# yigolden/JpegLibrary

Hardware: AMD Instinct MI355X
Metric: Mpixels/s decoded, 4K 4:2:0 baseline Q75 RST=4, 1 & 8 GPU vs CPU ref (higher is better)
Workload: dtype f32; 1 GPU; 1024 x 3840x2160 420 baseline Q75 DRI=4 per GPU, output interleaved_u8 resident in HBM; images_per_gpu=1024

## Files before the change

jpeglibrary_amd/csrc/common.h:

```cpp
#pragma once
#include <stdint.h>

namespace jpgpu {

constexpr int kMaxScanComponents = 4;
constexpr int kMaxBlocksPerMcu = 16;
constexpr int kHuffLutBits = 9;
constexpr int kHuffLutSize = 1 << kHuffLutBits;
constexpr int kMaxHuffSlots = 8;

struct alignas(16) DevHuffTable {
    uint16_t lut[kHuffLutSize];
    uint16_t maxcode[18];
    uint8_t valoffset[20];
    uint8_t values[256];
    uint8_t pad[8];
};
static_assert(sizeof(DevHuffTable) % 16 == 0, "DevHuffTable must be a multiple of 16 bytes");

struct alignas(16) DevQuantTable {
    uint16_t q[64];
};

struct DevScanComponent {
    uint8_t component_index;
    uint8_t h, v;
    uint8_t hs, vs;
    uint8_t quant_slot;
    uint8_t dc_slot, ac_slot;
};

enum OutputFormat : int32_t { kFmtInterleavedU8 = 0, kFmtPlanarU8 = 1, kFmtPlanarI16 = 2, kFmtRgbU8 = 3, kFmtRgbaU8 = 4, kFmtExtendedU16 = 5, kFmtInterleavedU8Scaled = 6, kFmtRgbPlanarU8 = 7, kFmtRgbPlanarF16 = 8, kFmtRgbPlanarF32 = 9 };
constexpr int kNumOutputFormats = 10;
constexpr bool fmt_is_sample_bytes(int f) { return f == kFmtInterleavedU8 || f == kFmtInterleavedU8Scaled; }
constexpr bool fmt_is_rgb_planes(int f) { return f == kFmtRgbPlanarU8 || f == kFmtRgbPlanarF16 || f == kFmtRgbPlanarF32; }
constexpr bool fmt_is_rgb(int f) { return f == kFmtRgbU8 || f == kFmtRgbaU8 || fmt_is_rgb_planes(f); }
constexpr int fmt_rgb_plane_sample_bytes(int f) { return f == kFmtRgbPlanarF16 ? 2 : (f == kFmtRgbPlanarF32 ? 4 : 1); }
constexpr bool fmt_is_interleaved(int f) { return fmt_is_sample_bytes(f) || fmt_is_rgb(f); }
constexpr int fmt_bytes_per_pixel_rgb(int f) { return f == kFmtRgbaU8 ? 4 : 3; }

struct YccRgbFactors {
    int32_t cr_r, cr_g, cb_b, cb_g;
};
struct OutputAffine {
    float scale[3], bias[3];
};
constexpr OutputAffine kOutputAffineIdentity = {{1.0f, 1.0f, 1.0f}, {0.0f, 0.0f, 0.0f}};
enum ColorKind : int32_t { kColorGray = 0, kColorYcbcr = 1, kColorRgb = 2, kColorCmyk = 3, kColorYcck = 4 };
constexpr bool color_kind_by_file(int k) { return k == kColorRgb || k == kColorCmyk || k == kColorYcck; }
constexpr int color_kind_sample_bytes(int k) { return k == kColorGray ? 1 : (k == kColorCmyk || k == kColorYcck ? 4 : 3); }

struct alignas(16) DevScan {
    uint64_t data_off;
    uint64_t coef_off;
    uint64_t out_off;
    uint64_t plane_off[kMaxScanComponents];
    uint32_t plane_pitch[kMaxScanComponents];
    uint32_t data_len;
    uint32_t dri;
    uint32_t total_mcus, mcus_per_line, mcus_per_column;
    uint32_t n_intervals;
    uint32_t ends_off;
    uint32_t image_index;
    uint32_t level_shift;
    uint16_t width, height;
    uint8_t precision, frame_components, scan_components, max_h, max_v, blocks_per_mcu;
    uint8_t restart_check_at_end;
    uint8_t shadow_mask;
    DevScanComponent comp[kMaxScanComponents];
    uint8_t blk_comp[kMaxBlocksPerMcu];
    uint8_t blk_x[kMaxBlocksPerMcu];
    uint8_t blk_y[kMaxBlocksPerMcu];
    uint16_t huff_pool[kMaxHuffSlots];
    uint16_t quant_pool[kMaxScanComponents];
    uint64_t reserved0;
// ... 132 lines not shown
```

jpeglibrary_amd/csrc/device_batch_layout.cpp:

```cpp
#include "device_batch.h"

#include <hip/hip_runtime.h>
#include <stdio.h>
#include <stdlib.h>
#include <string.h>

#include <algorithm>
#include <vector>

#include "kernels.h"

namespace jpgpu {

static inline uint64_t align_up(uint64_t v, uint64_t a) { return (v + a - 1) / a * a; }

namespace {
template <typename T>
void xcd_interleave(std::vector<T> &w, int xcds) {
    if (xcds <= 1 || w.size() < (size_t)xcds * 8) return;
    const size_t n = w.size(), per = (n + xcds - 1) / xcds;
    std::vector<T> m;
    m.reserve(n);
    for (size_t i = 0; m.size() < n; i++) {
        const size_t src = (i % xcds) * per + i / xcds;
        if (src < n) m.push_back(w[src]);
    }
    w.swap(m);
}

struct LayoutSwitches {
    int dbg_delay_scan = -1, dbg_delay_ms = 0;
    bool dbg_status = false, prog_no_pipeline = false, no_subseq = false;
    uint32_t subseq_shift = 0;
    uint32_t stream_max_intervals = 16;
    uint32_t prog_spin_budget = 1u << 17;
    bool subseq_host_check = false;
    bool handoff_set = false, handoff_dense = false;
    bool tile_align = true;
    bool overlap = false;
    int xcds = 8;
    bool prog_by_scan = false, no_wave_chains = false, k1_three_pass = false;
};

LayoutSwitches read_layout_switches() {
    auto set = [](const char *name) { return getenv(name) != nullptr; };
    static const bool by_scan = set("JPGPU_PROG_BY_SCAN"), no_wave_chains = set("JPGPU_PROG_NO_WAVE_CHAINS"), three_pass = set("JPGPU_K1_THREE_PASS");
    LayoutSwitches sw;
    const char *dd = getenv("JPGPU_DEBUG_DELAY_SCAN");
    if (dd && sscanf(dd, "%d:%d", &sw.dbg_delay_scan, &sw.dbg_delay_ms) != 2) sw.dbg_delay_scan = -1;
    sw.dbg_status = set("JPGPU_DEBUG_STATUS");
    if (const char *ev = getenv("JPGPU_SUBSEQ_SHIFT")) sw.subseq_shift = (uint32_t)std::min(14, std::max(8, atoi(ev)));
    if (const char *ev = getenv("JPGPU_PROG_STREAM_MAX_INTERVALS")) sw.stream_max_intervals = (uint32_t)atoi(ev);
    sw.prog_no_pipeline = set("JPGPU_PROG_NO_PIPELINE");
    if (const char *ev = getenv("JPGPU_PROG_SPIN_BUDGET")) sw.prog_spin_budget = (uint32_t)strtoul(ev, nullptr, 10);
    sw.subseq_host_check = set("JPGPU_SUBSEQ_HOST_CHECK");
    if (const char *ev = getenv("JPGPU_DENSE_HANDOFF")) sw.handoff_set = true, sw.handoff_dense = atoi(ev) != 0;
    if (const char *ev = getenv("JPGPU_TILE_ALIGN")) sw.tile_align = atoi(ev) != 0;
    sw.no_subseq = set("JPGPU_NO_SUBSEQ");
    if (const char *ev = getenv("JPGPU_OVERLAP")) sw.overlap = atoi(ev) != 0;
    if (const char *ev = getenv("JPGPU_XCD_MAP")) sw.xcds = atoi(ev);
    sw.prog_by_scan = by_scan, sw.no_wave_chains = no_wave_chains, sw.k1_three_pass = three_pass;
    return sw;
// ... 99 lines not shown
    sub_same_valid_ = k2s_unchecked_ = k2s_idct_behind_ = false;
    k2s_host_checked_ = p.sw.subseq_host_check || keep_canvas_;
    dispose_jobs_.clear();
    split_scans_.clear();
    dispose_max_blocks_ = split_max_blocks_ = 0;
    dense_valid_ = dense_override_ = false;
    compressed_bytes_ = total_pixels_ = 0;
    for (uint32_t &b : k2_ticket_base_) b = 0;
    decodes_since_query_ = 0;
}

void DeviceBatch::choose_batch_shapes(UploadPlan &p) {
    uint64_t dri0_bits = 0;
    for (size_t j = 0; j < jobs_.size(); j++)
        if (jobs_[j].kind == kScanSequential && jobs_[j].geo.restart_interval == 0) dri0_bits += (uint64_t)jobs_[j].entropy_len * 8;
    while (p.subseq_shift < 12 && (dri0_bits >> p.subseq_shift) >= 500000u) p.subseq_shift++;
    while (p.subseq_shift > 9 && (dri0_bits >> p.subseq_shift) < 4096u) p.subseq_shift--;
    if (p.sw.subseq_shift) p.subseq_shift = p.sw.subseq_shift;
    uint64_t blocks = 0;
    for (const ScanJob &job : jobs_)
        if (job.kind != kScanProgressive) blocks += (uint64_t)job.geo.mcus_per_line * job.geo.mcus_per_column * (uint64_t)std::max(1, job.blocks_per_mcu);
    const uint64_t tiles = blocks / (uint64_t)kIdctBlocksPerWg + 1, want_wgs = 3ull * (uint64_t)(ctx_->num_cus > 0 ? ctx_->num_cus : 256);
    while (p.idct_tiles_per_wg > 1 && tiles / p.idct_tiles_per_wg < want_wgs) p.idct_tiles_per_wg /= 2;
    n_huff_slots_ = 1;
    for (const ScanJob &job : jobs_) n_huff_slots_ = std::max(n_huff_slots_, job.n_huff);
    k2_tab_bytes_ = kK2AcTabBytes + kK2DcTabBytes;
    for (const ScanJob &job : jobs_) {
        if (job.kind != kScanSequential) continue;
        uint32_t bytes = 0;
        for (int k = 0; k < job.n_huff; k++) {
            bool is_dc = false;
            for (int c = 0; c < job.scan_components; c++) is_dc |= job.dc_slot[c] == k;
            bytes += is_dc ? kK2DcTabBytes : kK2AcTabBytes;
        }
        k2_tab_bytes_ = std::max(k2_tab_bytes_, bytes);
    }
    p.huff_intervals_per_wg = 64u * (uint32_t)huffman_waves(k2_tab_bytes_);
}

uint16_t DeviceBatch::huff_index(UploadPlan &p, const HuffTable &t) {
    for (size_t i = 0; i < p.huff_keys.size(); i++)
        if (p.huff_keys[i]->num_values == t.num_values && memcmp(p.huff_keys[i]->bits, t.bits, 16) == 0 &&
            memcmp(p.huff_keys[i]->values, t.values, t.num_values) == 0)
            return (uint16_t)i;
    DevHuffTable d;
    t.to_device(&d);
    p.huff_keys.push_back(&t);
    huff_pool_.push_back(d);
    return (uint16_t)(huff_pool_.size() - 1);
}
uint16_t DeviceBatch::quant_index(const QuantTable &t) {
    DevQuantTable d;
    memcpy(d.q, t.elements, sizeof d.q);
    for (size_t i = 0; i < quant_pool_.size(); i++)
        if (memcmp(&quant_pool_[i], &d, sizeof d) == 0) return (uint16_t)i;
    quant_pool_.push_back(d);
    return (uint16_t)(quant_pool_.size() - 1);
}

void DeviceBatch::plan_image(UploadPlan &p, size_t ii, const std::vector<size_t> &file_len) {
    ImagePlan &img = images_[ii];
    img.out_offset = p.out_off;
    img.planes_offset = p.planes_off;
    img.coef_offset = p.coef_off;
    img.total_blocks = 0;
    if (img.status != JPGPU_OK) return;
    p.out_off = align_up(p.out_off + slot_bytes(img), 256);
    p.planes_off = align_up(p.planes_off + img.planes_bytes, 256);
    if (!img.jobs.empty()) total_pixels_ += (uint64_t)img.width * img.height;
    bool overlapping_scans = false;
    uint32_t seen = 0;
    for (int j : img.jobs) {
        const ScanJob &job = jobs_[j];
        if (job.kind != kScanSequential || job.disabled) continue;
        overlapping_scans |= (component_mask(job) & seen) != 0;
        seen |= component_mask(job);
    }
    for (int j : img.jobs) {
        const ScanJob &job = jobs_[j];
        fill_scan(p, ii, j, file_len[ii]);
        if (job.kind == kScanFrameOnly && job.dispose_generic) plan_dispose_job(j, !img.replay_skip);
        if (job.kind == kScanProgressive) {
            if (!job.disabled && !img.replay_skip) plan_progressive_scan(p, img, j);
            continue;
        }
        plan_entropy_work(p, ii, j);
        if (img.replay_skip) continue;
        if (h_scans_[j].blocks_per_mcu == 0) continue;
        plan_idct_work(p, ii, j, overlapping_scans);
    }
}

void DeviceBatch::fill_scan(UploadPlan &p, size_t ii, int j, size_t file_len) {
    const ImagePlan &img = images_[ii];
    const ScanJob &job = jobs_[j];
    DevScan &s = h_scans_[j];
    memset(&s, 0, sizeof s);
    const BaselineGeometry &g = job.geo;
    s.kind = (uint8_t)job.kind;
    s.last_interval = job.last_interval;
    s.data_off = img.file_offset + job_entropy_off_[j];
    s.data_len = (uint32_t)(file_len - job_entropy_off_[j]);
    if (job.kind == kScanFrameOnly) s.data_len = 0;
    if (job.kind == kScanProgressive) {
        const size_t end = find_scan_end(job.entropy, job.entropy_len);
        s.data_len = (uint32_t)std::min<size_t>(end + 2, job.entropy_len);
// ... 594 lines not shown
```

jpeglibrary_amd/csrc/k3_idct.hip:

```cpp
#include <hip/hip_runtime.h>
#include <stdint.h>

#include <algorithm>
#include <atomic>
#include <cstdio>
#include <cstdlib>

#include "common.h"
#include "kernels.h"
#include "encode_kernels.h"
#include "kernels_device.h"
#include "k3_index_math.h"
#include "k3_store_quads.h"

namespace jpgpu {


__device__ constexpr uint8_t kNat[64] = {0,  1,  8,  16, 9,  2,  3,  10, 17, 24, 32, 25, 18, 11, 4,  5,  12, 19, 26, 33, 40, 48,
                                         41, 34, 27, 20, 13, 6,  7,  14, 21, 28, 35, 42, 49, 56, 57, 50, 43, 36, 29, 22, 15, 23,
                                         30, 37, 44, 51, 58, 59, 52, 45, 38, 31, 39, 46, 53, 60, 61, 54, 47, 55, 62, 63};

static_assert(kIdctBlocksPerWg == 256, "the split form's reciprocals are exact for tiles of up to 256 blocks");
static_assert(kMaxBlocksPerMcu == 16, "kRecip16 and the 16-bit reciprocals of the split form cover 1..16 blocks per MCU");
__device__ constexpr uint32_t kRecip16[kMaxBlocksPerMcu + 1] = {0, 65536, 32768, 21846, 16384, 13108, 10923, 9363, 8192, 7282, 6554, 5958, 5462, 5042, 4682, 4370, 4096};

#define JPGPU_IDCT8(y0, y1, y2, y3, y4, y5, y6, y7)                     \
    {                                                                   \
        float mz0 = y1 + y7;                                            \
        float mz2 = y3 + y7;                                            \
        float mz1 = y3 + y5;                                            \
        float mz3 = y1 + y5;                                            \
        float mz4 = (mz0 + mz1) * 1.175875602f;                         \
        mz2 = (mz2 * -1.961570560f) + mz4;                              \
        mz3 = (mz3 * -0.390180644f) + mz4;                              \
        mz0 = mz0 * -0.899976223f;                                      \
        mz1 = mz1 * -2.562915447f;                                      \
        const float mb3 = ((y7 * 0.298631336f) + mz0) + mz2;            \
        const float mb2 = ((y5 * 2.053119869f) + mz1) + mz3;            \
        const float mb1 = ((y3 * 3.072711026f) + mz1) + mz2;            \
        const float mb0 = ((y1 * 1.501321110f) + mz0) + mz3;            \
        mz4 = (y2 + y6) * 0.541196100f;                                 \
        mz0 = y0 + y4;                                                  \
        mz1 = y0 - y4;                                                  \
        mz2 = mz4 + (y6 * -1.847759065f);                               \
        mz3 = mz4 + (y2 * 0.765366865f);                                \
        const float a0 = mz0 + mz3;                                     \
        const float a3 = mz0 - mz3;                                     \
        const float a1 = mz1 + mz2;                                     \
        const float a2 = mz1 - mz2;                                     \
        y0 = a0 + mb0;                                                  \
        y7 = a0 - mb0;                                                  \
        y1 = a1 + mb1;                                                  \
        y6 = a1 - mb1;                                                  \
        y2 = a2 + mb2;                                                  \
        y5 = a2 - mb2;                                                  \
        y3 = a3 + mb3;                                                  \
        y4 = a3 - mb3;                                                  \
    }

__device__ __forceinline__ void block_dequant(const uint8_t *c_lds, uint32_t swz, const uint16_t *q_lds, float (&f)[64]) {
#pragma unroll
    for (int piece = 0; piece < 8; piece++) {
        const uint4 cv = *reinterpret_cast<const uint4 *>(c_lds + ((piece ^ swz) * 16));
        const uint4 qv = reinterpret_cast<const uint4 *>(q_lds)[piece];
        const uint32_t cw[4] = {cv.x, cv.y, cv.z, cv.w};
        const uint32_t qw[4] = {qv.x, qv.y, qv.z, qv.w};
#pragma unroll
        for (int j = 0; j < 8; j++) {
            const int k = piece * 8 + j;
            const uint32_t w = cw[j >> 1], q = qw[j >> 1];
            const int32_t c = (j & 1) ? ((int32_t)w >> 16) : (int32_t)(int16_t)(w & 0xFFFF);
            const int32_t qq = (j & 1) ? (int32_t)(q >> 16) : (int32_t)(q & 0xFFFF);
            f[kNat[k]] = (float)(qq * c);
        }
    }
}

typedef float float2v __attribute__((ext_vector_type(2)));
typedef short short2v __attribute__((ext_vector_type(2)));
typedef unsigned short ushort2v __attribute__((ext_vector_type(2)));

template <typename T>
__device__ __forceinline__ void idct8(T &y0, T &y1, T &y2, T &y3, T &y4, T &y5, T &y6, T &y7) {
    T mz0 = y1 + y7;
    T mz2 = y3 + y7;
    T mz1 = y3 + y5;
    T mz3 = y1 + y5;
    T mz4 = (mz0 + mz1) * 1.175875602f;
    mz2 = (mz2 * -1.961570560f) + mz4;
    mz3 = (mz3 * -0.390180644f) + mz4;
    mz0 = mz0 * -0.899976223f;
    mz1 = mz1 * -2.562915447f;
    const T mb3 = ((y7 * 0.298631336f) + mz0) + mz2;
    const T mb2 = ((y5 * 2.053119869f) + mz1) + mz3;
    const T mb1 = ((y3 * 3.072711026f) + mz1) + mz2;
    const T mb0 = ((y1 * 1.501321110f) + mz0) + mz3;
    mz4 = (y2 + y6) * 0.541196100f;
    mz0 = y0 + y4;
    mz1 = y0 - y4;
    mz2 = mz4 + (y6 * -1.847759065f);
    mz3 = mz4 + (y2 * 0.765366865f);
    const T a0 = mz0 + mz3;
    const T a3 = mz0 - mz3;
    const T a1 = mz1 + mz2;
    const T a2 = mz1 - mz2;
    y0 = a0 + mb0;
    y7 = a0 - mb0;
    y1 = a1 + mb1;
    y6 = a1 - mb1;
    y2 = a2 + mb2;
    y5 = a2 - mb2;
    y3 = a3 + mb3;
    y4 = a3 - mb3;
}

__device__ __forceinline__ void block_idct(const float (&f)[64], int32_t level_shift, uint32_t (&out)[32]) {
#if defined(JPGPU_K3_PRICE)
#pragma unroll
    for (int i = 0; i < 32; i++) out[i] = (__builtin_bit_cast(uint32_t, f[2 * i]) >> 16) | (__builtin_bit_cast(uint32_t, f[2 * i + 1]) & 0xFFFF0000u) | (uint32_t)level_shift;
    return;
#endif
    float2v a[4][8];
#pragma unroll
    for (int r2 = 0; r2 < 4; r2++)
#pragma unroll
        for (int c = 0; c < 8; c++) a[r2][c] = float2v{f[(2 * r2) * 8 + c], f[(2 * r2 + 1) * 8 + c]};
#pragma unroll
    for (int r2 = 0; r2 < 4; r2++) idct8(a[r2][0], a[r2][1], a[r2][2], a[r2][3], a[r2][4], a[r2][5], a[r2][6], a[r2][7]);
    float2v b[8][4];
#pragma unroll
    for (int r2 = 0; r2 < 4; r2++)
#pragma unroll
        for (int c2 = 0; c2 < 4; c2++) {
            b[2 * r2][c2] = float2v{a[r2][2 * c2].x, a[r2][2 * c2 + 1].x};
            b[2 * r2 + 1][c2] = float2v{a[r2][2 * c2].y, a[r2][2 * c2 + 1].y};
        }
#pragma unroll
    for (int c2 = 0; c2 < 4; c2++) idct8(b[0][c2], b[1][c2], b[2][c2], b[3][c2], b[4][c2], b[5][c2], b[6][c2], b[7][c2]);
    const uint32_t shift2 = ((uint32_t)level_shift & 0xFFFFu) * 0x00010001u;
#pragma unroll
    for (int r = 0; r < 8; r++)
#pragma unroll
        for (int c2 = 0; c2 < 4; c2++) {
            const float2v v = b[r][c2] * 0.1250f;
            const int32_t x = (int32_t)__builtin_rintf(v.x);
            const int32_t y = (int32_t)__builtin_rintf(v.y);
            const uint32_t pk = ((uint32_t)x & 0xFFFFu) | ((uint32_t)y << 16);
            const short2v sum = __builtin_bit_cast(short2v, pk) + __builtin_bit_cast(short2v, shift2);
            out[r * 4 + c2] = __builtin_bit_cast(uint32_t, sum);
        }
}

__device__ __forceinline__ uint32_t clamp2_u8(uint32_t pk) {
    short2v v = __builtin_bit_cast(short2v, pk);
    v = __builtin_elementwise_max(v, short2v{0, 0});
    v = __builtin_elementwise_min(v, short2v{255, 255});
    return __builtin_bit_cast(uint32_t, v);
}
__device__ __forceinline__ uint32_t pack4_u8(uint32_t pk01, uint32_t pk23) {
    return __builtin_amdgcn_perm(clamp2_u8(pk23), clamp2_u8(pk01), 0x06040200u);
}
struct ScaleTo8 {
    uint32_t shift2, max2, mul2, rem2, mask2;
    bool expand;
};
__device__ __forceinline__ ScaleTo8 scale_to_8(uint32_t precision) {
    const uint32_t p = precision < 1u ? 1u : (precision > 16u ? 16u : precision);
    ScaleTo8 k;
    k.expand = p < 8u;
    const uint32_t pe = k.expand ? p : 1u;
    const uint32_t m = (uint32_t)(0x010101110955FFull >> (8u * (pe - 1u))) & 0xFFu;
    const uint32_t rem = 8u % pe;
    k.shift2 = (k.expand ? 0u : p - 8u) * 0x00010001u;
    k.max2 = ((1u << pe) - 1u) * 0x00010001u;
    k.mul2 = m * 0x00010001u;
    k.rem2 = rem * 0x00010001u;
    k.mask2 = ((1u << rem) - 1u) * 0x00010001u;
    return k;
}
__device__ __forceinline__ uint32_t shift_sat2_u8(uint32_t pk, const ScaleTo8 &k) {
    const uint32_t t = __builtin_bit_cast(uint32_t, __builtin_bit_cast(short2v, pk) >> __builtin_bit_cast(short2v, k.shift2));
    uint32_t r;
    asm("v_sat_pk_u8_i16 %0, %1" : "=v"(r) : "v"(t));
    return r;
}
__device__ __forceinline__ uint32_t expand2_u8(uint32_t pk, const ScaleTo8 &k) {
    short2v v = __builtin_bit_cast(short2v, pk);
    v = __builtin_elementwise_max(v, short2v{0, 0});
    v = __builtin_elementwise_min(v, __builtin_bit_cast(short2v, k.max2));
    const ushort2v r = __builtin_bit_cast(ushort2v, v) * __builtin_bit_cast(ushort2v, k.mul2);
    const ushort2v hi = r << __builtin_bit_cast(ushort2v, k.rem2);
    return __builtin_bit_cast(uint32_t, hi) | (__builtin_bit_cast(uint32_t, r) & k.mask2);
}
__device__ __forceinline__ uint32_t pick4(uint32_t lo, uint32_t hi, uint32_t sel) { return __builtin_amdgcn_perm(hi, lo, sel); }
#define JPGPU_SEL(a, b, c, d) ((uint32_t)(a) | ((uint32_t)(b) << 8) | ((uint32_t)(c) << 16) | ((uint32_t)(d) << 24))

constexpr int kIdctThreads = 256;
constexpr uint32_t kPxRowStride = kIdctThreads * 8;

enum IdctLayout : int { kLayGeneric = 0, kLayYccH1V1 = 1, kLayYccH2V1 = 2, kLayYccH2V2 = 3, kLayGray = 4, kNumIdctLayouts = 5 };

struct ChromaTerms {
    int32_t r, g, b;
};
__device__ __forceinline__ ChromaTerms chroma_terms(uint32_t cb_sample, uint32_t cr_sample, const YccRgbFactors &k) {
    const int32_t cb = (int32_t)cb_sample - 128, cr = (int32_t)cr_sample - 128;
    ChromaTerms t;
    t.r = (k.cr_r * cr + 32768) >> 16;
    t.b = (k.cb_b * cb + 32768) >> 16;
    t.g = (k.cb_g * cb + 32768 + k.cr_g * cr) >> 16;
    return t;
}
__device__ __forceinline__ uint32_t clamp_u8_i32(int32_t v) { return (uint32_t)(v < 0 ? 0 : (v > 255 ? 255 : v)); }
// ... 346 lines not shown
            o2.y = pick4(yv.w, cc3, JPGPU_SEL(0, 4, 5, 1));
            o2.z = pick4(yv.w, cc3, JPGPU_SEL(4, 5, 2, 6));
            o2.w = pick4(yv.w, cc3, JPGPU_SEL(7, 3, 6, 7));
            if (kQuads) {
                uint4 d0, d1, d2;
                quad_exchange(o0, o1, o2, keep, d0, d1, d2);
                *reinterpret_cast<uint4 *>(line0 + (at + q_off[0])) = d0;
                *reinterpret_cast<uint4 *>(line0 + (at + q_off[1])) = d1;
                *reinterpret_cast<uint4 *>(line0 + (at + q_off[2])) = d2;
            } else {
                uint4 *dst = reinterpret_cast<uint4 *>(dst_px);
                dst[0] = o0;
                dst[1] = o1;
                dst[2] = o2;
            }
        } else {
            const uint2 yv = *reinterpret_cast<const uint2 *>(yrow);
            const uint2 bv = *reinterpret_cast<const uint2 *>(crow);
            const uint2 rv = *reinterpret_cast<const uint2 *>(crow + 8);
            uint2 o0, o1, o2;
            {
                const uint32_t lo = pick4(bv.x, rv.x, JPGPU_SEL(0, 4, 1, 5)), hi = pick4(bv.x, rv.x, JPGPU_SEL(2, 6, 3, 7));
                const uint32_t mid = pick4(lo, hi, JPGPU_SEL(2, 3, 4, 5));
                o0.x = pick4(yv.x, lo, JPGPU_SEL(0, 4, 5, 1));
                o0.y = pick4(yv.x, mid, JPGPU_SEL(4, 5, 2, 6));
                o1.x = pick4(yv.x, hi, JPGPU_SEL(5, 3, 6, 7));
            }
            {
                const uint32_t lo = pick4(bv.y, rv.y, JPGPU_SEL(0, 4, 1, 5)), hi = pick4(bv.y, rv.y, JPGPU_SEL(2, 6, 3, 7));
                const uint32_t mid = pick4(lo, hi, JPGPU_SEL(2, 3, 4, 5));
                o1.y = pick4(yv.y, lo, JPGPU_SEL(0, 4, 5, 1));
                o2.x = pick4(yv.y, mid, JPGPU_SEL(4, 5, 2, 6));
                o2.y = pick4(yv.y, hi, JPGPU_SEL(5, 3, 6, 7));
            }
            uint2 *dst = reinterpret_cast<uint2 *>(dst_px);
            dst[0] = o0;
            dst[1] = o1;
            dst[2] = o2;
        }
    }
    }
}

typedef __attribute__((address_space(3))) void jpgpu_lds_void;
typedef const __attribute__((address_space(1))) void jpgpu_gbl_void;

template <int FMT, int LAY, bool PRE, bool SPLIT = false, bool WIN = false>
__device__ __forceinline__ void idct_output_body(
    const int16_t *__restrict__ coefs, const DevScan *__restrict__ scans, const IdctWork *__restrict__ work,
    const DevScanStatus *__restrict__ status, const DevQuantTable *__restrict__ quant_pool, uint8_t *__restrict__ out, YccRgbFactors kf,
    OutputAffine aff = kOutputAffineIdentity) {
    constexpr int CONV = FMT == kFmtRgbU8 ? 3 : (FMT == kFmtRgbaU8 ? 4 : (FMT == kFmtRgbPlanarU8 ? kConvPlanar : (FMT == kFmtRgbPlanarF16 ? kConvPlanarF16 : (FMT == kFmtRgbPlanarF32 ? kConvPlanarF32 : 0))));
    constexpr bool kSampleBytes = fmt_is_sample_bytes(FMT);
    __shared__ __attribute__((aligned(16))) uint8_t sh_all[kIdctThreads * 128 + kIdctThreads * 64 + kMaxScanComponents * 128 + (SPLIT && !PRE ? 64 : 0)];
    uint8_t *sh = sh_all;
    uint8_t *sh_px = sh_all + kIdctThreads * 128;
    uint16_t(*sh_q)[64] = reinterpret_cast<uint16_t(*)[64]>(sh_all + kIdctThreads * 128 + kIdctThreads * 64);
    uint8_t *sh_flag = sh_all + kIdctThreads * 128 + kIdctThreads * 64 + kMaxScanComponents * 128;

    const IdctWork wk = work[blockIdx.x];
    const DevScan &s = scans[wk.scan];
    const uint32_t tid = threadIdx.x;
    const uint32_t wave = tid >> 6;
    const uint32_t bpm = s.blocks_per_mcu;
    const uint32_t mcus_per_tile = wk.mcus_per_tile;
    uint32_t decoded = status ? status[wk.scan].decoded_mcus : s.total_mcus;
    if (decoded > s.total_mcus) decoded = s.total_mcus;
    uint32_t fail_block = 0xFFFFFFFFu;
    if (status != nullptr && s.kind == kScanSequential) {
        const uint32_t fb = status[wk.scan].pad[1];
        if (fb != 0) fail_block = kFailBlockBase - fb;
        for (uint32_t j = s.first_scan; j < wk.scan; j++)
            if (scans[j].image_index == s.image_index && status[j].first_error != kNoError) fail_block = 0;
    }
    const bool keep = (s.shadow_mask & kKeepUnreachedMcus) != 0;
    constexpr bool kPerMcuLayout = fmt_is_interleaved(FMT) && (LAY == kLayYccH1V1 || LAY == kLayYccH2V1 || LAY == kLayYccH2V2);
    uint32_t first_mcu = wk.first_mcu;
    uint32_t range_end = wk.first_mcu + wk.n_mcus;
    const bool win_whole = !WIN || (s.cov_x == 0 && s.cov_y == 0 && s.cov_cols == s.mcus_per_line);
    if (!WIN && first_mcu == kIdctPartialMcu) {
        if (fail_block == 0xFFFFFFFFu || fail_block % bpm == 0 || fail_block / bpm >= decoded) return;
        first_mcu = fail_block / bpm;
        range_end = first_mcu + 1;
    } else if (keep && win_whole) {
        const uint32_t reach = kPerMcuLayout ? fail_block / bpm : (fail_block == 0xFFFFFFFFu ? fail_block : (fail_block + bpm - 1) / bpm);
        if (range_end > decoded) range_end = decoded;
        if (range_end > reach) range_end = reach;
        if (first_mcu >= range_end) return;
    }

    if (tid < (uint32_t)s.scan_components * 32) {
        const uint32_t c = tid >> 5, i = tid & 31;
        reinterpret_cast<uint32_t *>(sh_q[c])[i] =
            reinterpret_cast<const uint32_t *>(quant_pool[s.quant_pool[s.comp[c].quant_slot]].q)[i];
    }

    const uint32_t mcu_local = tid / bpm;
    const uint32_t b = tid - mcu_local * bpm;
    const uint32_t ci_early = s.blk_comp[b < kMaxBlocksPerMcu ? b : 0];
    const uint8_t *coef_bytes = reinterpret_cast<const uint8_t *>(coefs + s.coef_off * 64);

    auto tile_mcus = [&](uint32_t first) { return (range_end - first) < mcus_per_tile ? (range_end - first) : mcus_per_tile; };
    const uint32_t tile_blocks = mcus_per_tile * bpm;
    static_assert(!(WIN && SPLIT), "a windowed image's scans are handed over dense");
    constexpr bool split = SPLIT && !PRE;
    if (split && (s.reserved0 & kScanSplitHandoff) == 0) return;
    const uint32_t sp_dri = split ? s.dri : 1u;
    const uint32_t sp_rb = kRecip16[bpm <= (uint32_t)kMaxBlocksPerMcu ? bpm : 0];
    const uint32_t sp_rd = __builtin_amdgcn_readfirstlane(sp_dri <= 256u ? ((1u << 20) + sp_dri - 1) / sp_dri : 0u);
    const uint32_t sp_w = sp_dri * bpm;
    const bool sp_fast = split && mcus_per_tile % (2 * sp_dri) == 0 && first_mcu % (2 * sp_dri) == 0;
    const uint32_t sp_rw = __builtin_amdgcn_readfirstlane((65536u + sp_w - 1) / sp_w);
    const uint8_t *sp_hi = coef_bytes + split_plane_lines(s.n_intervals, sp_dri, bpm) * 128;
    const uint8_t *sp_flags = reinterpret_cast<const uint8_t *>(reinterpret_cast<const uint64_t *>(coefs) + (s.reserved0 >> kSplitFlagShift));
    auto sp_locate = [&](uint32_t tile_first, uint32_t t, uint32_t k, uint32_t &line, uint32_t &iv, uint32_t &word) {
        const uint32_t i0 = __builtin_amdgcn_readfirstlane(tile_first / sp_dri), m0 = tile_first - i0 * sp_dri;
        const uint32_t blk = k * 32 + (t >> 3);
        uint32_t q = (blk * sp_rb) >> 16;
        const uint32_t bb = blk - q * bpm;
        const uint32_t last = s.total_mcus - 1 - tile_first;
        q = q < last ? q : last;
        const uint32_t mm = m0 + q;
        const uint32_t by_mul = (mm * sp_rd) >> 20, by_cmp = mm >= sp_dri ? 1u : 0u;
        const uint32_t qi = sp_dri > 256u ? by_cmp : by_mul;
        const uint32_t m = mm - qi * sp_dri;
        iv = i0 + qi;
        line = ((iv >> 1) * sp_dri + m) * bpm + bb;
        word = ((iv >> 6) * sp_dri + m) * bpm + bb;
    };
    auto sp_locate_fast = [&](uint32_t i0, uint32_t t, uint32_t k, uint32_t &iv, uint32_t &word) {
        const uint32_t ll = k * 16 + ((t >> 3) & 15u);
        const uint32_t pp = (ll * sp_rw) >> 16;
        iv = i0 + 2 * pp + ((t >> 7) & 1u);
        iv = iv < s.n_intervals ? iv : s.n_intervals - 1;
        word = (iv >> 6) * sp_w + (ll - pp * sp_w);
    };
    auto sp_own_block = [&](uint32_t t) {
        const uint32_t ml = (t * sp_rb) >> 16, bb = t - ml * bpm;
        const uint32_t ir = (ml * sp_rd) >> 20, m = ml - ir * sp_dri;
        const uint32_t ll = ((ir >> 1) * sp_dri + m) * bpm + bb;
        return ((ll >> 4) << 5) | ((ir & 1u) << 4) | (ll & 15u);
    };
    const uint32_t sp_ipt = __builtin_amdgcn_readfirstlane(mcus_per_tile / sp_dri);
    uint32_t sp_i0 = __builtin_amdgcn_readfirstlane(first_mcu / sp_dri);
    auto sp_load_flag = [&](uint32_t tile_first, uint32_t tile_i0, uint32_t &fb, uint32_t &bit_at) {
        uint32_t t_ = tid;
        asm volatile("" : "+v"(t_));
// ... 81 lines not shown
            const uint32_t mx = s.cov_x + cx - k3_mul24(wr, win_mpl), my = s.cov_y + tp.gy0 + wr;
            const uint32_t block = (my * s.mcus_per_line + mx) * bpm + bb;
            if (k < 6 || blk < tile_blocks)
                __builtin_amdgcn_global_load_lds((jpgpu_gbl_void *)(coef_bytes + (uint64_t)block * 128 + piece_off),
                                                 (jpgpu_lds_void *)(sh + ((uint32_t)k * kIdctThreads + wave * 64) * 16), 16, 0, 0);
        }
    };

    uint32_t hi_next = 0;
    if (WIN) {
        dma_tile_win(k3_tile_pos(first_mcu, win_mpl), first_mcu);
    } else if (split) {
        const uint32_t n_sets = first_mcu + mcus_per_tile < range_end ? 2u : 1u;
#pragma nounroll
        for (uint32_t set = 0; set < n_sets; set++) {
            uint32_t fb, at;
            sp_load_flag(first_mcu + set * mcus_per_tile, sp_i0 + set * sp_ipt, fb, at);
            asm volatile("s_waitcnt vmcnt(0)" ::: "memory");
            sp_wait_seen();
            sp_publish_flags(fb, at, set);
        }
        __syncthreads();
        const uint32_t hi_first = sp_read_flags(0);
        if (n_sets == 2) hi_next = sp_read_flags(1);
        dma_tile(first_mcu, sp_i0, hi_first);
    } else {
        dma_tile(first_mcu, sp_i0, 0);
    }
    const uint32_t mpl = WIN ? win_mpl : __builtin_amdgcn_readfirstlane(s.mcus_per_line);
    const uint32_t line_recip = WIN ? win_recip : __builtin_amdgcn_readfirstlane(k3_line_recip(mpl));
    const uint32_t img_h = __builtin_amdgcn_readfirstlane(WIN ? (uint32_t)s.win_h : (uint32_t)s.height);
    uint8_t *const img = out + s.out_off;
    K3TilePos pos = k3_tile_pos(first_mcu, mpl);
    pos.gx0 = __builtin_amdgcn_readfirstlane(pos.gx0);
    pos.gy0 = __builtin_amdgcn_readfirstlane(pos.gy0);
    K3TilePos pos_step = k3_tile_pos(mcus_per_tile, mpl);
    pos_step.gx0 = __builtin_amdgcn_readfirstlane(pos_step.gx0);
    pos_step.gy0 = __builtin_amdgcn_readfirstlane(pos_step.gy0);
    const uint32_t row_recip_full = __builtin_amdgcn_readfirstlane(k3_row_recip(mcus_per_tile));
    const uint32_t row_recip_last = __builtin_amdgcn_readfirstlane(k3_row_recip((range_end - first_mcu - 1) % mcus_per_tile + 1));
    asm volatile("s_waitcnt vmcnt(0)" ::: "memory");
    __syncthreads();

  for (uint32_t tile_first = first_mcu; tile_first < range_end; tile_first += mcus_per_tile) {
    const uint32_t n_mcu = tile_mcus(tile_first);
    const uint32_t n_blk = n_mcu * bpm;
    const uint32_t next_first = tile_first + mcus_per_tile;
    const bool have_next = next_first < range_end;

    uint32_t mcu = tile_first + mcu_local;
    const bool have_block = tid < n_blk;
    bool writes = have_block && ((s.shadow_mask >> ci_early) & 1u) == 0;

    float f[64];
    uint32_t px[32];
    if (PRE) {
        if (have_block) {
#pragma unroll
            for (int piece = 0; piece < 8; piece++) {
                const uint4 cv = *reinterpret_cast<const uint4 *>(sh + tid * 128 + ((piece ^ ((tid >> 1) & 7)) * 16));
                px[piece * 4] = cv.x;
                px[piece * 4 + 1] = cv.y;
                px[piece * 4 + 2] = cv.z;
                px[piece * 4 + 3] = cv.w;
            }
        }
    } else {
        constexpr bool kPerTile = split || (FMT == kFmtRgbU8 && (LAY == kLayYccH2V1 || LAY == kLayYccH2V2)) || (kSampleBytes && LAY == kLayGeneric);
        uint32_t t_ = tid;
        if (kPerTile) asm volatile("" : "+v"(t_));
        if (split && sp_fast) t_ = sp_own_block(t_);
        if (have_block) block_dequant(sh + t_ * 128, (t_ >> 1) & 7, sh_q[ci_early], f);
    }
    asm volatile("s_waitcnt lgkmcnt(0)" ::: "memory");
    __builtin_amdgcn_s_barrier();
    if (WIN) {
        K3TilePos pos_next = pos;
        k3_tile_advance(pos_next, pos_step, mpl);
        if (have_next) dma_tile_win(pos_next, next_first);
    } else if (have_next) dma_tile(next_first, sp_i0 + sp_ipt, hi_next);
    hi_next = 0;

    if (!PRE && have_block) block_idct(f, (int32_t)s.level_shift, px);
    uint32_t sp_fb = 0, sp_at = 0;
    const bool sp_ahead = split && next_first + mcus_per_tile < range_end;
    if (sp_ahead) sp_load_flag(next_first + mcus_per_tile, sp_i0 + 2 * sp_ipt, sp_fb, sp_at);
    sp_i0 += sp_ipt;
    uint32_t win_mx = 0, win_my = 0;
    if (WIN) {
        uint32_t ml_win = mcu_local;
        asm volatile("" : "+v"(ml_win));
        const uint32_t wr = k3_line_wraps(pos.gx0 + ml_win, mpl, line_recip);
        win_mx = s.cov_x + pos.gx0 + ml_win - k3_mul24(wr, mpl);
        win_my = s.cov_y + pos.gy0 + wr;
        mcu = win_my * s.mcus_per_line + win_mx;
    }
    const bool reached = mcu < decoded && mcu * bpm + b < fail_block;
    if ((s.shadow_mask & 0xFu) == 0) {
        writes = writes && (reached || !keep);
    } else {
        const uint32_t bb = b < kMaxBlocksPerMcu ? b : 0u, me = s.blk_comp[bb], fc = s.comp[me & 3u].component_index;
        uint32_t later = 0xFFu, earlier = 0xFFu;
        for (uint32_t cc = 0; cc < s.scan_components && cc < (uint32_t)kMaxScanComponents; cc++) {
            if (cc == me || s.comp[cc].component_index != fc) continue;
            if (cc > me && later == 0xFFu) later = cc;
            if (cc < me) earlier = cc;
        }
        uint32_t first_me = 0xFFu, first_later = 0xFFu, first_earlier = 0xFFu;
        for (uint32_t k = 0; k < bpm && k < (uint32_t)kMaxBlocksPerMcu; k++) {
            const uint32_t ck = s.blk_comp[k];
            if (ck == me && first_me == 0xFFu) first_me = k;
            if (ck == later && first_later == 0xFFu) first_later = k;
            if (ck == earlier && first_earlier == 0xFFu) first_earlier = k;
        }
        const bool later_reached = later != 0xFFu && mcu < decoded && mcu * bpm + (b - first_me + first_later) < fail_block;
        const bool earlier_reached = earlier != 0xFFu && mcu < decoded && mcu * bpm + (b - first_me + first_earlier) < fail_block;
        writes = have_block && (reached ? !later_reached : (!keep && later == 0xFFu && !earlier_reached));
    }
    if (!reached) {
#pragma unroll
        for (int i = 0; i < 32; i++) px[i] = 0;
    }
    bool synced = false;
    uint32_t ml_late = mcu_local, b_late = b;
    asm volatile("" : "+v"(ml_late), "+v"(b_late));
    const uint32_t mcu_wraps = k3_line_wraps(pos.gx0 + ml_late, mpl, line_recip);
    uint32_t mcu_back = k3_mul24(mcu_wraps, mpl);
    asm("" : "+v"(mcu_back));
    const uint32_t mcu_y = WIN ? win_my : pos.gy0 + mcu_wraps, mcu_x = WIN ? win_mx : pos.gx0 + ml_late - mcu_back;
    const uint32_t ci = s.blk_comp[b_late < kMaxBlocksPerMcu ? b_late : 0];
    const DevScanComponent comp = s.comp[ci];
    const uint32_t b_out = split ? b_late : b;

    if (FMT == kFmtPlanarI16) {
        if (writes) {
            int16_t *plane = reinterpret_cast<int16_t *>(out + s.out_off + s.plane_off[ci]);
// ... 138 lines not shown
}
template <int FMT, int LAY>
__global__ __launch_bounds__(kIdctThreads, (FMT == kFmtPlanarI16 ? 2 : 3)) void idct_split_kernel(
    const int16_t *__restrict__ coefs, const DevScan *__restrict__ scans, const IdctWork *__restrict__ work,
    const DevScanStatus *__restrict__ status, const DevQuantTable *__restrict__ quant_pool, uint8_t *__restrict__ out, YccRgbFactors kf, OutputAffine aff) {
    idct_output_body<FMT, LAY, false, true>(coefs, scans, work, status, quant_pool, out, kf, aff);
}
template <int FMT>
__global__ __launch_bounds__(kIdctThreads, 2) void flush_output_kernel(
    const int16_t *__restrict__ coefs, const DevScan *__restrict__ scans, const IdctWork *__restrict__ work,
    const DevScanStatus *__restrict__ status, const DevQuantTable *__restrict__ quant_pool, uint8_t *__restrict__ out, YccRgbFactors kf) {
    idct_output_body<FMT, kLayGeneric, true>(coefs, scans, work, status, quant_pool, out, kf);
}

template <int FMT, int LAY>
__global__ __launch_bounds__(kIdctThreads, 3) void idct_window_kernel(
    const int16_t *__restrict__ coefs, const DevScan *__restrict__ scans, const IdctWork *__restrict__ work,
    const DevScanStatus *__restrict__ status, const DevQuantTable *__restrict__ quant_pool, uint8_t *__restrict__ out, YccRgbFactors kf, OutputAffine aff) {
    idct_output_body<FMT, LAY, false, false, true>(coefs, scans, work, status, quant_pool, out, kf, aff);
}
template <int FMT>
__global__ __launch_bounds__(kIdctThreads, 2) void flush_window_kernel(
    const int16_t *__restrict__ coefs, const DevScan *__restrict__ scans, const IdctWork *__restrict__ work,
    const DevScanStatus *__restrict__ status, const DevQuantTable *__restrict__ quant_pool, uint8_t *__restrict__ out, YccRgbFactors kf) {
    idct_output_body<FMT, kLayGeneric, true, false, true>(coefs, scans, work, status, quant_pool, out, kf);
}

__global__ __launch_bounds__(64) void dispose_pass_kernel(int16_t *__restrict__ coefs, const DisposeJob *__restrict__ jobs,
                                                          const DevQuantTable *__restrict__ quant_pool) {
    const DisposeJob &j = jobs[blockIdx.y];
    const uint32_t g = blockIdx.x * 64u + threadIdx.x;
    if (g >= j.n_blocks) return;
    const uint32_t c = j.blk_comp[g % j.bpm];
    const uint32_t n = j.n[c];
    if (n == 0) return;
    int16_t *blk = coefs + (j.coef_off + g) * 64;
    uint32_t w[32];
#pragma unroll
    for (int i = 0; i < 8; i++) {
        const uint4 v = reinterpret_cast<const uint4 *>(blk)[i];
        w[i * 4] = v.x;
        w[i * 4 + 1] = v.y;
        w[i * 4 + 2] = v.z;
        w[i * 4 + 3] = v.w;
    }
    for (uint32_t t = 0; t < n; t++) {
        const uint16_t *q = quant_pool[j.quant[c][t]].q;
        float f[64];
#pragma unroll
        for (int k = 0; k < 64; k++) {
            const int32_t cv = (k & 1) ? ((int32_t)w[k >> 1] >> 16) : (int32_t)(int16_t)(w[k >> 1] & 0xFFFFu);
            f[kNat[k]] = (float)((int32_t)q[k] * cv);
        }
        block_idct(f, (int32_t)j.level_shift, w);
    }
#pragma unroll
    for (int i = 0; i < 8; i++) reinterpret_cast<uint4 *>(blk)[i] = make_uint4(w[i * 4], w[i * 4 + 1], w[i * 4 + 2], w[i * 4 + 3]);
}

template <int FMT, int LAY>
static void launch_idct_one(hipStream_t stream, const int16_t *coefs, const DevScan *scans, const IdctWork *work, int n_work, int n_dense,
                            const DevScanStatus *status, const DevQuantTable *quant_pool, uint8_t *out,
                            YccRgbFactors kf = YccRgbFactors{0, 0, 0, 0}, OutputAffine aff = kOutputAffineIdentity) {
    if (n_dense > 0)
        hipLaunchKernelGGL((idct_output_kernel<FMT, LAY>), dim3(n_dense), dim3(kIdctThreads), 0, stream, coefs, scans, work, status,
                           quant_pool, out, kf, aff);
    if constexpr (idct_split_supported(FMT, LAY))
      if (n_work > n_dense)
        hipLaunchKernelGGL((idct_split_kernel<FMT, LAY>), dim3(n_work - n_dense), dim3(kIdctThreads), 0, stream, coefs, scans, work + n_dense, status,
                           quant_pool, out, kf, aff);
}

template <int FMT>
static void launch_window_fast(hipStream_t stream, int c, const int16_t *coefs, const DevScan *scans, const IdctWork *w, int n, const DevScanStatus *status,
                               const DevQuantTable *quant_pool, uint8_t *out, const YccRgbFactors &kf, const OutputAffine &aff) {
    switch (c) {
    case kLayYccH1V1: hipLaunchKernelGGL((idct_window_kernel<FMT, kLayYccH1V1>), dim3(n), dim3(kIdctThreads), 0, stream, coefs, scans, w, status, quant_pool, out, kf, aff); break;
    case kLayYccH2V1: hipLaunchKernelGGL((idct_window_kernel<FMT, kLayYccH2V1>), dim3(n), dim3(kIdctThreads), 0, stream, coefs, scans, w, status, quant_pool, out, kf, aff); break;
    case kLayYccH2V2: hipLaunchKernelGGL((idct_window_kernel<FMT, kLayYccH2V2>), dim3(n), dim3(kIdctThreads), 0, stream, coefs, scans, w, status, quant_pool, out, kf, aff); break;
    default: hipLaunchKernelGGL((idct_window_kernel<FMT, kLayGray>), dim3(n), dim3(kIdctThreads), 0, stream, coefs, scans, w, status, quant_pool, out, kf, aff); break;
    }
}

hipError_t launch_idct_window(hipStream_t stream, const int16_t *coefs, const DevScan *scans, const IdctWork *work,
                              const int class_begin[kNumIdctLayoutClasses + 1], const DevScanStatus *status, const DevQuantTable *quant_pool, uint8_t *out,
                              int format, const YccRgbFactors &kf, uint8_t *generic_out, const OutputAffine &aff) {
    if (!fmt_is_interleaved(format)) return class_begin[kNumIdctLayoutClasses] > class_begin[0] ? hipErrorInvalidValue : hipSuccess;
    const bool scaled = format == kFmtInterleavedU8Scaled;
    uint8_t *const bytes_out = fmt_is_rgb(format) ? generic_out : out;
    for (int c = 0; c < kNumIdctLayoutClasses; c++) {
        const int n = class_begin[c + 1] - class_begin[c];
        if (n <= 0) continue;
        const IdctWork *w = work + class_begin[c];
        const bool fast = c >= kLayYccH1V1 && c <= kLayGray;
        if (c == kIdctClassStoreHoldsSamples) {
            if (scaled) hipLaunchKernelGGL((flush_window_kernel<kFmtInterleavedU8Scaled>), dim3(n), dim3(kIdctThreads), 0, stream, coefs, scans, w, status, quant_pool, bytes_out, kf);
            else hipLaunchKernelGGL((flush_window_kernel<kFmtInterleavedU8>), dim3(n), dim3(kIdctThreads), 0, stream, coefs, scans, w, status, quant_pool, bytes_out, kf);
        } else if (fast && format == kFmtRgbU8) {
            launch_window_fast<kFmtRgbU8>(stream, c, coefs, scans, w, n, status, quant_pool, out, kf, aff);
        } else if (fast && format == kFmtRgbPlanarU8) {
            launch_window_fast<kFmtRgbPlanarU8>(stream, c, coefs, scans, w, n, status, quant_pool, out, kf, aff);
        } else if (fast && format == kFmtRgbPlanarF16) {
            launch_window_fast<kFmtRgbPlanarF16>(stream, c, coefs, scans, w, n, status, quant_pool, out, kf, aff);
        } else if (fast && format == kFmtRgbPlanarF32) {
            launch_window_fast<kFmtRgbPlanarF32>(stream, c, coefs, scans, w, n, status, quant_pool, out, kf, aff);
        } else if (c != kLayGeneric) {
            return hipErrorInvalidValue;
// ... 143 lines not shown
```

Measured before the change: 654,800 Mpixels/s.

## Fold dequantisation and IDCT scaling into float quant tables in pair order

```diff
diff --git a/jpeglibrary_amd/csrc/common.h b/jpeglibrary_amd/csrc/common.h
--- a/jpeglibrary_amd/csrc/common.h
+++ b/jpeglibrary_amd/csrc/common.h
@@ -20,7 +20,9 @@
 
 struct alignas(16) DevQuantTable {
     uint16_t q[64];
-};
+    float qf[64];
+};
+static_assert(sizeof(DevQuantTable) == 128 + 256, "DevQuantTable has no padding: the pool finds duplicates with memcmp");
 
 struct DevScanComponent {
     uint8_t component_index;
diff --git a/jpeglibrary_amd/csrc/device_batch_layout.cpp b/jpeglibrary_amd/csrc/device_batch_layout.cpp
--- a/jpeglibrary_amd/csrc/device_batch_layout.cpp
+++ b/jpeglibrary_amd/csrc/device_batch_layout.cpp
@@ -8,6 +8,7 @@
 #include <algorithm>
 #include <vector>
 
+#include "k3_quant_order.h"
 #include "kernels.h"
 
 namespace jpgpu {
@@ -213,6 +214,7 @@
 uint16_t DeviceBatch::quant_index(const QuantTable &t) {
     DevQuantTable d;
     memcpy(d.q, t.elements, sizeof d.q);
+    k3_quant_pair_floats(d.q, d.qf);
     for (size_t i = 0; i < quant_pool_.size(); i++)
         if (memcmp(&quant_pool_[i], &d, sizeof d) == 0) return (uint16_t)i;
     quant_pool_.push_back(d);
diff --git a/jpeglibrary_amd/csrc/k3_idct.hip b/jpeglibrary_amd/csrc/k3_idct.hip
--- a/jpeglibrary_amd/csrc/k3_idct.hip
+++ b/jpeglibrary_amd/csrc/k3_idct.hip
@@ -11,6 +11,7 @@
 #include "encode_kernels.h"
 #include "kernels_device.h"
 #include "k3_index_math.h"
+#include "k3_quant_order.h"
 #include "k3_store_quads.h"
 
 namespace jpgpu {
@@ -58,22 +59,27 @@
         y4 = a3 - mb3;                                                  \
     }
 
-__device__ __forceinline__ void block_dequant(const uint8_t *c_lds, uint32_t swz, const uint16_t *q_lds, float (&f)[64]) {
+constexpr bool zig_of_nat_inverts_nat() {
+    for (int k = 0; k < 64; k++)
+        if (kZigOfNat[kNat[k]] != k) return false;
+    return true;
+}
+static_assert(zig_of_nat_inverts_nat(), "k3_quant_order.h's kZigOfNat is the inverse of kNat");
+
+__device__ __forceinline__ void block_load(const uint8_t *c_lds, uint32_t swz, uint32_t (&cw)[32]) {
 #pragma unroll
     for (int piece = 0; piece < 8; piece++) {
         const uint4 cv = *reinterpret_cast<const uint4 *>(c_lds + ((piece ^ swz) * 16));
-        const uint4 qv = reinterpret_cast<const uint4 *>(q_lds)[piece];
-        const uint32_t cw[4] = {cv.x, cv.y, cv.z, cv.w};
-        const uint32_t qw[4] = {qv.x, qv.y, qv.z, qv.w};
-#pragma unroll
-        for (int j = 0; j < 8; j++) {
-            const int k = piece * 8 + j;
-            const uint32_t w = cw[j >> 1], q = qw[j >> 1];
-            const int32_t c = (j & 1) ? ((int32_t)w >> 16) : (int32_t)(int16_t)(w & 0xFFFF);
-            const int32_t qq = (j & 1) ? (int32_t)(q >> 16) : (int32_t)(q & 0xFFFF);
-            f[kNat[k]] = (float)(qq * c);
-        }
-    }
+        cw[piece * 4] = cv.x;
+        cw[piece * 4 + 1] = cv.y;
+        cw[piece * 4 + 2] = cv.z;
+        cw[piece * 4 + 3] = cv.w;
+    }
+}
+__device__ __forceinline__ float coef_at(const uint32_t (&cw)[32], int n) {
+    const int k = kZigOfNat[n];
+    const uint32_t w = cw[k >> 1];
+    return (float)((k & 1) ? ((int32_t)w >> 16) : (int32_t)(int16_t)(w & 0xFFFFu));
 }
 
 typedef float float2v __attribute__((ext_vector_type(2)));
@@ -114,26 +120,14 @@
     y4 = a3 - mb3;
 }
 
-__device__ __forceinline__ void block_idct(const float (&f)[64], int32_t level_shift, uint32_t (&out)[32]) {
-#if defined(JPGPU_K3_PRICE)
-#pragma unroll
-    for (int i = 0; i < 32; i++) out[i] = (__builtin_bit_cast(uint32_t, f[2 * i]) >> 16) | (__builtin_bit_cast(uint32_t, f[2 * i + 1]) & 0xFFFF0000u) | (uint32_t)level_shift;
-    return;
-#endif
-    float2v a[4][8];
+__device__ __forceinline__ void idct_columns_out(const float2v (&a)[4][8], int32_t level_shift, uint32_t (&out)[32]) {
+    float2v b[8][4];
 #pragma unroll
     for (int r2 = 0; r2 < 4; r2++)
 #pragma unroll
-        for (int c = 0; c < 8; c++) a[r2][c] = float2v{f[(2 * r2) * 8 + c], f[(2 * r2 + 1) * 8 + c]};
-#pragma unroll
-    for (int r2 = 0; r2 < 4; r2++) idct8(a[r2][0], a[r2][1], a[r2][2], a[r2][3], a[r2][4], a[r2][5], a[r2][6], a[r2][7]);
-    float2v b[8][4];
-#pragma unroll
-    for (int r2 = 0; r2 < 4; r2++)
-#pragma unroll
         for (int c2 = 0; c2 < 4; c2++) {
-            b[2 * r2][c2] = float2v{a[r2][2 * c2].x, a[r2][2 * c2 + 1].x};
-            b[2 * r2 + 1][c2] = float2v{a[r2][2 * c2].y, a[r2][2 * c2 + 1].y};
+            asm("v_pk_mov_b32 %0, %1, %2 op_sel:[0,0] op_sel_hi:[0,0]" : "=v"(b[2 * r2][c2]) : "v"(a[r2][2 * c2]), "v"(a[r2][2 * c2 + 1]));
+            asm("v_pk_mov_b32 %0, %1, %2 op_sel:[1,1] op_sel_hi:[1,1]" : "=v"(b[2 * r2 + 1][c2]) : "v"(a[r2][2 * c2]), "v"(a[r2][2 * c2 + 1]));
         }
 #pragma unroll
     for (int c2 = 0; c2 < 4; c2++) idct8(b[0][c2], b[1][c2], b[2][c2], b[3][c2], b[4][c2], b[5][c2], b[6][c2], b[7][c2]);
@@ -142,7 +136,7 @@
     for (int r = 0; r < 8; r++)
 #pragma unroll
         for (int c2 = 0; c2 < 4; c2++) {
-            const float2v v = b[r][c2] * 0.1250f;
+            const float2v v = b[r][c2];
             const int32_t x = (int32_t)__builtin_rintf(v.x);
             const int32_t y = (int32_t)__builtin_rintf(v.y);
             const uint32_t pk = ((uint32_t)x & 0xFFFFu) | ((uint32_t)y << 16);
@@ -151,14 +145,53 @@
         }
 }
 
+__device__ __forceinline__ void block_idct(const uint32_t (&cw)[32], const float *q_lds, int32_t level_shift, uint32_t (&out)[32]) {
+    float2v a[4][8];
+#pragma unroll
+    for (int r2 = 0; r2 < 4; r2++) {
+#pragma unroll
+        for (int c = 0; c < 8; c += 2) {
+            const float4 q = reinterpret_cast<const float4 *>(q_lds)[r2 * 4 + (c >> 1)];
+            a[r2][c] = float2v{coef_at(cw, (2 * r2) * 8 + c), coef_at(cw, (2 * r2 + 1) * 8 + c)} * float2v{q.x, q.y};
+            a[r2][c + 1] = float2v{coef_at(cw, (2 * r2) * 8 + c + 1), coef_at(cw, (2 * r2 + 1) * 8 + c + 1)} * float2v{q.z, q.w};
+        }
+#if !defined(JPGPU_K3_PRICE)
+        idct8(a[r2][0], a[r2][1], a[r2][2], a[r2][3], a[r2][4], a[r2][5], a[r2][6], a[r2][7]);
+#endif
+    }
+#if defined(JPGPU_K3_PRICE)
+#pragma unroll
+    for (int i = 0; i < 32; i++)
+        out[i] = (__builtin_bit_cast(uint32_t, a[i >> 3][i & 7].x) >> 16) | (__builtin_bit_cast(uint32_t, a[i >> 3][i & 7].y) & 0xFFFF0000u) | (uint32_t)level_shift;
+    return;
+#endif
+    idct_columns_out(a, level_shift, out);
+}
+
+__device__ __forceinline__ void block_idct_dequantised(const float (&f)[64], int32_t level_shift, uint32_t (&out)[32]) {
+    float2v a[4][8];
+#pragma unroll
+    for (int r2 = 0; r2 < 4; r2++) {
+#pragma unroll
+        for (int c = 0; c < 8; c++) a[r2][c] = float2v{f[(2 * r2) * 8 + c], f[(2 * r2 + 1) * 8 + c]} * 0.125f;
+        idct8(a[r2][0], a[r2][1], a[r2][2], a[r2][3], a[r2][4], a[r2][5], a[r2][6], a[r2][7]);
+    }
+    idct_columns_out(a, level_shift, out);
+}
+
 __device__ __forceinline__ uint32_t clamp2_u8(uint32_t pk) {
     short2v v = __builtin_bit_cast(short2v, pk);
     v = __builtin_elementwise_max(v, short2v{0, 0});
     v = __builtin_elementwise_min(v, short2v{255, 255});
     return __builtin_bit_cast(uint32_t, v);
 }
+__device__ __forceinline__ uint32_t sat2_u8(uint32_t pk) {
+    uint32_t r;
+    asm("v_sat_pk_u8_i16 %0, %1" : "=v"(r) : "v"(pk));
+    return r;
+}
 __device__ __forceinline__ uint32_t pack4_u8(uint32_t pk01, uint32_t pk23) {
-    return __builtin_amdgcn_perm(clamp2_u8(pk23), clamp2_u8(pk01), 0x06040200u);
+    return __builtin_amdgcn_perm(sat2_u8(pk23), sat2_u8(pk01), 0x05040100u);
 }
 struct ScaleTo8 {
     uint32_t shift2, max2, mul2, rem2, mask2;
@@ -611,11 +644,11 @@
     OutputAffine aff = kOutputAffineIdentity) {
     constexpr int CONV = FMT == kFmtRgbU8 ? 3 : (FMT == kFmtRgbaU8 ? 4 : (FMT == kFmtRgbPlanarU8 ? kConvPlanar : (FMT == kFmtRgbPlanarF16 ? kConvPlanarF16 : (FMT == kFmtRgbPlanarF32 ? kConvPlanarF32 : 0))));
     constexpr bool kSampleBytes = fmt_is_sample_bytes(FMT);
-    __shared__ __attribute__((aligned(16))) uint8_t sh_all[kIdctThreads * 128 + kIdctThreads * 64 + kMaxScanComponents * 128 + (SPLIT && !PRE ? 64 : 0)];
+    __shared__ __attribute__((aligned(16))) uint8_t sh_all[kIdctThreads * 128 + kIdctThreads * 64 + kMaxScanComponents * 256 + (SPLIT && !PRE ? 64 : 0)];
     uint8_t *sh = sh_all;
     uint8_t *sh_px = sh_all + kIdctThreads * 128;
-    uint16_t(*sh_q)[64] = reinterpret_cast<uint16_t(*)[64]>(sh_all + kIdctThreads * 128 + kIdctThreads * 64);
-    uint8_t *sh_flag = sh_all + kIdctThreads * 128 + kIdctThreads * 64 + kMaxScanComponents * 128;
+    float(*sh_q)[64] = reinterpret_cast<float(*)[64]>(sh_all + kIdctThreads * 128 + kIdctThreads * 64);
+    uint8_t *sh_flag = sh_all + kIdctThreads * 128 + kIdctThreads * 64 + kMaxScanComponents * 256;
 
     const IdctWork wk = work[blockIdx.x];
     const DevScan &s = scans[wk.scan];
@@ -648,10 +681,10 @@
         if (first_mcu >= range_end) return;
     }
 
-    if (tid < (uint32_t)s.scan_components * 32) {
-        const uint32_t c = tid >> 5, i = tid & 31;
-        reinterpret_cast<uint32_t *>(sh_q[c])[i] =
-            reinterpret_cast<const uint32_t *>(quant_pool[s.quant_pool[s.comp[c].quant_slot]].q)[i];
+    static_assert(kMaxScanComponents * 64 <= kIdctThreads, "one lane per table entry");
+    if (tid < (uint32_t)s.scan_components * 64) {
+        const uint32_t c = tid >> 6, i = tid & 63;
+        sh_q[c][i] = quant_pool[s.quant_pool[s.comp[c].quant_slot]].qf[i];
     }
 
     const uint32_t mcu_local = tid / bpm;
@@ -839,7 +872,7 @@
     const bool have_block = tid < n_blk;
     bool writes = have_block && ((s.shadow_mask >> ci_early) & 1u) == 0;
 
-    float f[64];
+    uint32_t cw[32];
     uint32_t px[32];
     if (PRE) {
         if (have_block) {
@@ -857,7 +890,7 @@
         uint32_t t_ = tid;
         if (kPerTile) asm volatile("" : "+v"(t_));
         if (split && sp_fast) t_ = sp_own_block(t_);
-        if (have_block) block_dequant(sh + t_ * 128, (t_ >> 1) & 7, sh_q[ci_early], f);
+        if (have_block) block_load(sh + t_ * 128, (t_ >> 1) & 7, cw);
     }
     asm volatile("s_waitcnt lgkmcnt(0)" ::: "memory");
     __builtin_amdgcn_s_barrier();
@@ -868,7 +901,7 @@
     } else if (have_next) dma_tile(next_first, sp_i0 + sp_ipt, hi_next);
     hi_next = 0;
 
-    if (!PRE && have_block) block_idct(f, (int32_t)s.level_shift, px);
+    if (!PRE && have_block) block_idct(cw, sh_q[ci_early], (int32_t)s.level_shift, px);
     uint32_t sp_fb = 0, sp_at = 0;
     const bool sp_ahead = split && next_first + mcus_per_tile < range_end;
     if (sp_ahead) sp_load_flag(next_first + mcus_per_tile, sp_i0 + 2 * sp_ipt, sp_fb, sp_at);
@@ -1113,7 +1146,7 @@
             const int32_t cv = (k & 1) ? ((int32_t)w[k >> 1] >> 16) : (int32_t)(int16_t)(w[k >> 1] & 0xFFFFu);
             f[kNat[k]] = (float)((int32_t)q[k] * cv);
         }
-        block_idct(f, (int32_t)j.level_shift, w);
+        block_idct_dequantised(f, (int32_t)j.level_shift, w);
     }
 #pragma unroll
     for (int i = 0; i < 8; i++) reinterpret_cast<uint4 *>(blk)[i] = make_uint4(w[i * 4], w[i * 4 + 1], w[i * 4 + 2], w[i * 4 + 3]);
diff --git a/jpeglibrary_amd/csrc/k3_quant_order.h b/jpeglibrary_amd/csrc/k3_quant_order.h
--- /dev/null
+++ b/jpeglibrary_amd/csrc/k3_quant_order.h
@@ -0,0 +1,15 @@
+#pragma once
+#include <stdint.h>
+
+namespace jpgpu {
+
+constexpr uint8_t kZigOfNat[64] = {0,  1,  5,  6,  14, 15, 27, 28, 2,  4,  7,  13, 16, 26, 29, 42, 3,  8,  12, 17, 25, 30, 41, 43, 9,  11, 18, 24, 31, 40, 44, 53,
+                                   10, 19, 23, 32, 39, 45, 52, 54, 20, 22, 33, 38, 46, 51, 55, 60, 21, 34, 37, 47, 50, 56, 59, 61, 35, 36, 48, 49, 57, 58, 62, 63};
+
+constexpr int k3_pair_order_nat(int e) { return (2 * (e >> 4) + (e & 1)) * 8 + ((e >> 1) & 7); }
+
+inline void k3_quant_pair_floats(const uint16_t (&q)[64], float (&qf)[64]) {
+    for (int e = 0; e < 64; e++) qf[e] = (float)q[kZigOfNat[k3_pair_order_nat(e)]] * 0.125f;
+}
+
+}
```

Measured after the change: 673,900 Mpixels/s, median of 6. +2.9%, better.
